# yassram/iterative-closest-point

Measured on AMD Instinct MI355X. Metric: ICP iterations/sec (synthetic 1048576-point pair, C4, exact NN), higher is better.
Workload: dtype f64 (30 exact fp64 grid searches (fp32 screen, candidates decided in fp64: the first from cell seeds, the seeded ones the fused grid iteration nn_grid_iter2_kernel, 75% of its queries kept their correspondence by the exclusion certificate without a walk); fp64 transform and reductions)

## Files before the change

### iterative-closest-point_amd/csrc/icp_canon.hip

```cpp
#include <hip/hip_runtime.h>

#include <cstdlib>

#include "icp_bundle_rec.h"
#include "icp_canon.h"
#include "icp_device.h"
#include "icp_fold.h"
#include "icp_gridbox.h"
#include "icp_kernels.h"
#include "icp_mfma16.h"

namespace icp {
namespace {

template <int K>
__device__ __forceinline__ void strands_to_row(const double (&acc)[K], double *__restrict__ rows, int R)
{
    __shared__ double sh[kBlock / 64][K];
    const int lane = threadIdx.x & 63, wave = threadIdx.x >> 6;
    if (lane == 0)
#pragma unroll
        for (int k = 0; k < K; ++k) sh[wave][k] = acc[k];
    __syncthreads();
    if (threadIdx.x < K) {
// ... 194 lines not shown
        const int k = threadIdx.x;
        double s[kFoldThreads / 64];
#pragma unroll
        for (int w = 0; w < kFoldThreads / 64; ++w) s[w] = sh[w][k];
#pragma unroll
        for (int span = 1; span < kFoldThreads / 64; span <<= 1)
#pragma unroll
            for (int w = 0; w < kFoldThreads / 64; w += 2 * span) s[w] = s[w] + s[w + span];
        sums[K0 + k] = s[0];
        s_sum[K0 + k] = s[0];
    }
    if (MODE == 0 && K0 == 0 && K == kCanonCols && threadIdx.x == 0)
        sums[kSumFar] = (double)__hip_atomic_load(&cs.s->far_acc, __ATOMIC_RELAXED, __HIP_MEMORY_SCOPE_AGENT);
    if constexpr (MODE == 0) return;
    __syncthreads();
    if (threadIdx.x != 0) return;
    if constexpr (MODE != 4)
        err_step_body(s_sum, cs.N, cs.threshold, cs.max_iter, cs.err_trace, cs.s, cs.hflag, cs.ticket, cs.h_state,
                      cs.h_trace);
    if constexpr (MODE == 1 || MODE == 4) horn_step_body(s_sum, cs.N, cs.c[0], cs.c[1], cs.c[2], 1, cs.cnt, cs.s);
}


template <int MODE>
__global__ __launch_bounds__(kFoldThreads) void canon_fold_cols_kernel(const double *__restrict__ rows, int R,
                                                                       double *__restrict__ sums, CanonStep cs, int S)
{
    __shared__ double sh[kFoldThreads / 64];
    __shared__ double s_sum[kCanonCols];
    __shared__ int s_last;
    const int lane = threadIdx.x & 63, wave = threadIdx.x >> 6, k = blockIdx.x;
    const double *col = rows + (size_t)k * (S > 0 ? S : R);
    double a = 0.0;
    constexpr int U = 4;
    for (int r0 = threadIdx.x; r0 < R; r0 += U * kFoldThreads) {
        double v[U];
#pragma unroll
        for (int u = 0; u < U; ++u) {
            const int r = r0 + u * kFoldThreads;
            v[u] = r < R ? canon_row_value(col, S, r) : 0.0;
        }
#pragma unroll
        for (int u = 0; u < U; ++u)
            if (r0 + u * kFoldThreads < R) a = a + v[u];
    }
    const double w = wave_tree_halves(a);
    const double two = lane_value(w, 31) + lane_value(w, 63);
    if (lane == 0) sh[wave] = two;
    __syncthreads();
    if (threadIdx.x == 0) {
// ... 30 lines not shown
                          int n, double *yx, double *yy, double *yz, const IterState *st_dev, double *rows,
                          hipStream_t st, const int *kpos, const double4 *m4kd, bool y_ready)
{
    if (n <= 0) return;
    const int R = canon_rows((size_t)n);
    if (y_ready)
        canon_moments_kernel<true><<<R, kBlock, 0, st>>>(idx, m4, px, py, pz, n, yx, yy, yz, st_dev, rows, kpos, m4kd);
    else
        canon_moments_kernel<false><<<R, kBlock, 0, st>>>(idx, m4, px, py, pz, n, yx, yy, yz, st_dev, rows, kpos, m4kd);
}

void launch_canon_transform(double *px, double *py, double *pz, const double *yx, const double *yy, const double *yz,
                            int n, const Xform *xf, const int *done, float4 *p32, double *rows, const SeedArgs &sa,
                            hipStream_t st)
{
    if (n <= 0) return;
    const int R = canon_rows((size_t)n);
    if (sa.qop)
        canon_transform_kernel<true><<<R, kBlock, 0, st>>>(px, py, pz, yx, yy, yz, n, xf, done, p32, rows, sa);
    else
        canon_transform_kernel<false><<<R, kBlock, 0, st>>>(px, py, pz, yx, yy, yz, n, xf, done, p32, rows, sa);
}

void launch_canon_fold(const double *rows, int n, double *sums, int mode, const CanonStep &cs, hipStream_t st,
                       int strands)
{
    const int R = canon_rows((size_t)(n > 0 ? n : 1));
    static const bool one = [] {
        const char *e = getenv("ICP_FOLD_ONE");
        return e && atoi(e) == 1;
    }();
    if (!one && cs.fold_ticket && (mode == 0 || mode == 1 || mode == 4)) {
        if (mode == 0) canon_fold_cols_kernel<0><<<kCanonCols, kFoldThreads, 0, st>>>(rows, R, sums, cs, strands);
        else if (mode == 1) canon_fold_cols_kernel<1><<<kCanonCols, kFoldThreads, 0, st>>>(rows, R, sums, cs, strands);
        else canon_fold_cols_kernel<4><<<kCanonCols, kFoldThreads, 0, st>>>(rows, R, sums, cs, strands);
        return;
    }
    switch (mode) {
    case 0: canon_fold_kernel<0, kCanonCols, 0><<<1, kFoldThreads, 0, st>>>(rows, R, sums, cs, strands); break;
    case 1: canon_fold_kernel<0, kCanonCols, 1><<<1, kFoldThreads, 0, st>>>(rows, R, sums, cs, strands); break;
    case 4: canon_fold_kernel<0, kCanonCols, 4><<<1, kFoldThreads, 0, st>>>(rows, R, sums, cs, strands); break;
    case 2: canon_fold_kernel<kSumErr, 1, 2><<<1, kFoldThreads, 0, st>>>(rows, R, sums, cs, strands); break;
    default: canon_fold_kernel<kSumErr, 1, 0><<<1, kFoldThreads, 0, st>>>(rows, R, sums, cs, strands); break;
    }
}

}
```

### iterative-closest-point_amd/csrc/icp_engine.h

```cpp
#pragma once

#include <hip/hip_runtime.h>
#include <rccl/rccl.h>

#include <string>
#include <vector>

#include "icp_canon.h"
#include "icp_kernels.h"

namespace icp {
namespace engine {

struct DevCloud {
    double *x = nullptr, *y = nullptr, *z = nullptr;
    float4 *f = nullptr;
    size_t n = 0, cap = 0;
};

}
}

using namespace icp;
using namespace icp::engine;
// ... 236 lines not shown
    bool seedd = false;
    int seed16 = 0;
    bool records = false;
    double rec_local = -1.0;
};

struct RunKnobs {
    int grid_budget;
    bool grid_auto, grid_iter;
    int grid_xcd;
    bool bundle_order_off, scene_order_off, cell_seed, first_k1;
    int run_mode;
    bool persist_mid_off, persist_stamps;
    int persist_cull;
    bool mid_prepass, transform_records;
    int far_shift;
    bool far_dist;
    int fused_steps;
    bool err_pair;
    int timing_stride;
    bool canon, cert;
    int cert_two;
    double cert_skin, cert_skin1;
    int iter_debug;
    bool tail_split_err, debug_policy;
};
const RunKnobs &run_knobs();

struct RunTestKnobs {
    int enqueue_delay_us;
    bool tail_test_abort, persist_test_abort;
};
RunTestKnobs run_test_knobs();

constexpr int kSeededBox = 125;

int fail(icp_ctx *ctx, int code, const std::string &msg);

template <class T> int grow(icp_ctx *ctx, T **p, size_t *cap, size_t count)
{
    if (*cap >= count && *p) return ICP_OK;
    if (*p) HIPCHK(hipFree(*p));
    *p = nullptr;
    *cap = 0;
    size_t bytes = sizeof(T) * (count ? count : 1);
    HIPCHK(hipMalloc((void **)p, bytes));
// ... 28 lines not shown
```

### iterative-closest-point_amd/csrc/icp_grid.hip

```cpp
#include <hip/hip_runtime.h>

#include <algorithm>
#include <cmath>
#include <cstdlib>
#include <string>
#include <type_traits>

#include "icp_canon.h"
#include "icp_device.h"
#include "icp_gridbox.h"
#include "icp_kernels.h"

namespace icp {
namespace {

__device__ __forceinline__ double d64g(double px, double py, double pz, double mx, double my,
                                       double mz)
{
    const double dx = px - mx;
    const double dy = py - my;
    const double dz = pz - mz;
    return (dx * dx + dy * dy) + dz * dz;
}

// ... 449 lines not shown
        best = d;
        bi = mi;
        bk = k;
    }
}

template <int G> __device__ __forceinline__ void group_lex_min_pos(double &best, int &bi, int &bk)
{
#pragma unroll
    for (int o = G / 2; o >= 1; o >>= 1) {
        const double ob = __shfl_xor(best, o, G);
        const int oi = __shfl_xor(bi, o, G);
        const int ok = __shfl_xor(bk, o, G);
        if (ob < best || (ob == best && (unsigned)oi < (unsigned)bi)) {
            best = ob;
            bi = oi;
            bk = ok;
        } else if (ob == best && oi == bi) {
            bk = max(bk, ok);
        }
    }
}

__device__ __forceinline__ int xcd_row(int b, int nb, int L)
{
    const int k = b & 7, i = b >> 3;
    if (L < 0) {
        const int q = nb >> 3, e = nb & 7;
        return k * q + min(k, e) + i;
    }
    if (L == 0 || b >= nb / (8 * L) * (8 * L)) return b;
    return ((i / L) * 8 + k) * L + i % L;
}

template <int G, int KR, int KU, int W, int TB = kBlock>
__global__ __launch_bounds__(TB, W) void nn_grid_seeded_kernel(
    int n, const double *__restrict__ px, const double *__restrict__ py, const double *__restrict__ pz, GridView gv,
    int budget, const double *__restrict__ seedd, const double4 *__restrict__ m4, int *__restrict__ idx,
    double *__restrict__ yx, double *__restrict__ yy, double *__restrict__ yz, int *far_count,
    int *__restrict__ far_list, int *__restrict__ far_hint, const int *__restrict__ stop, int xcd_remap, int trim)
{
    if (stop && *stop) return;
    const int sub = threadIdx.x & (G - 1);
    const int groups = gridDim.x * (TB / G);
    const int bx = xcd_row((int)blockIdx.x, (int)gridDim.x, xcd_remap);
    for (int t = (bx * TB + threadIdx.x) / G; t < n; t += groups) {
        const int h = idx[t];
        const double q[3] = {px[t], py[t], pz[t]};
        double best = seedd[t];
        int bi = h, bk = -1, c0[3], c1[3];
        const bool ok = h >= 0 && best == best && best < INFINITY && complete_box(q, best, gv, budget, c0, c1);
        if (ok) {
            const int ny = c1[1] - c0[1] + 1;
            const int nrows = ny * (c1[2] - c0[2] + 1);
            for (int r0 = sub; r0 < nrows; r0 += KR * G) {
                int k0[KR], pre[KR + 1];
// ... 748 lines not shown
    auto *p = (const ICP_CONST_AS IterState *)st;
    asm volatile("" : "+s"(p));
    return *(const IterState *)p;
}

template <bool A32, class T> __device__ __forceinline__ T &at32(T *b, int i)
{
    if constexpr (A32) return *(T *)((char *)b + (unsigned)i * (unsigned)sizeof(T));
    else return b[i];
}

template <int KR, int KU, int CH, int NWG, bool A32>
__global__ __launch_bounds__(64 * NWG) __attribute__((amdgpu_waves_per_eu(ICP_ITER2_WAVES))) void nn_grid_iter2_kernel(
    Iter2Args args_)
{
    static_assert(CH == 1 || CH == 2, "one or two chunks a task");
    constexpr bool kDbg = ICP_ITER2_DBG != 0;
    unsigned long long dcnt[4] = {0, 0, 0, 0};
    static_assert(NWG == 4 || NWG == 1, "a row or a strand a workgroup");
    constexpr int NW = NWG, QL = 2 / CH;
    __shared__ double s_tile[NW][CH * kIter2Tile];
    const Iter2Args &T = iter2_args();
    const IterState *const st = T.st;
    if (iter2_state(st).done) return;
    const int n = T.n, xcd_l = T.xcd_l, xform = T.xform;
    const int lane = threadIdx.x & 63, wave = threadIdx.x >> 6, u = lane / QL, sub = lane % QL;
    const int C = canon_chunks((size_t)n), S = canon_strands((size_t)n), R = canon_rows((size_t)n);
    const int s = NWG == 4 ? xcd_row((int)blockIdx.x, R, xcd_l) * 4 + wave
                           : xcd_row((int)blockIdx.x, S, xcd_l > 0 ? 4 * xcd_l : xcd_l);
    const int wr = s >> 2;
    double *const tile = s_tile[wave];
    double *const slots = tile;
    int *const wl = (int *)(tile + 32 * CH * kIter2Slot);
    auto at = [](auto *b, int i) -> auto & { return at32<A32>(b, i); };
    const bool cert_on = T.ca.state != nullptr, cert_in = cert_on && T.ca.valid != 0, two = T.ca.two != 0;
    auto wave_sync = [] {
        __builtin_amdgcn_fence(__ATOMIC_RELEASE, "wavefront");
        __builtin_amdgcn_wave_barrier();
        __builtin_amdgcn_fence(__ATOMIC_ACQUIRE, "wavefront");
    };
    double acc = 0.0;
    int far = 0, nbig = 0, ncert = 0, nwalk = 0;
    auto slot_t = [&](int c, int uu) { return (c + (uu >> 5) * S) * kCanonChunk + (uu & 31); };
    for (int c = s; s < S && c < C; c += CH * S) {
        const int t = slot_t(c, u);
        const bool active = c + (u >> 5) * S < C && t < n;
        if (kDbg) dcnt[0] += 1;
        const Iter2Args &A = iter2_args();
        const Xform xf = iter2_state(st).xf;
        double *const px = A.px, *const py = A.py, *const pz = A.pz, *const yx = A.yx, *const yy = A.yy, *const yz = A.yz;
        int *const idx = A.idx;
        int4 *const cstate = A.ca.state;
// ... 417 lines not shown
        wave_sync();
        double tv = 0.0;
        if ((lane & 31) < kCanonCols && (CH == 2 || lane < 32)) {
            const double *col = tile + (lane >> 5) * kIter2Tile + (lane & 31) * kLeafStride;
            double part[4];
#pragma unroll
            for (int g8 = 0; g8 < 4; ++g8) {
                double v[8];
#pragma unroll
                for (int j = 0; j < 8; ++j) v[j] = col[8 * g8 + j];
                part[g8] = ((v[0] + v[1]) + (v[2] + v[3])) + ((v[4] + v[5]) + (v[6] + v[7]));
            }
            tv = (part[0] + part[1]) + (part[2] + part[3]);
        }
        const double tb = CH == 2 ? __shfl(tv, (lane & 31) + 32, 64) : 0.0;
        if (lane < kCanonCols) {
            acc = acc + tv;
            if (CH == 2 && c + S < C) acc = acc + tb;
        }
        wave_sync();
    }
    const Iter2Args &E = iter2_args();
    unsigned long long *const dbg = E.dbg;
    if (kDbg && dbg && lane == 0)
        for (int f = 0; f < 4; ++f)
            if (dcnt[f]) atomicAdd(dbg + f, dcnt[f]);
    if constexpr (NWG == 4) {
        __shared__ double sh[NW][kCanonCols];
        if (lane < kCanonCols) sh[wave][lane] = acc;
        __syncthreads();
        if (threadIdx.x < kCanonCols) {
            const int k = threadIdx.x;
            E.rows[(size_t)k * R + wr] = (sh[0][k] + sh[1][k]) + (sh[2][k] + sh[3][k]);
        }
    } else if (s < S && lane < kCanonCols) {
        E.rows[(size_t)lane * S + s] = acc;
    }
    __shared__ int s_cnt[4][NW];
    for (int o = 32; o >= 1; o >>= 1) {
        far += __shfl_xor(far, o, 64);
        ncert += __shfl_xor(ncert, o, 64);
        nwalk += __shfl_xor(nwalk, o, 64);
    }
    if (lane == 0) {
        s_cnt[0][wave] = far;
        s_cnt[1][wave] = nbig;
        s_cnt[2][wave] = ncert;
        s_cnt[3][wave] = nwalk;
    }
    __syncthreads();
    if (threadIdx.x < 4) {
        int tot = 0;
        for (int w = 0; w < NW; ++w) tot += s_cnt[threadIdx.x][w];
        if (threadIdx.x < 2) {
            int *dst = threadIdx.x == 0 ? E.far_acc : E.big_count;
            if (tot && dst) atomicAdd(dst, tot);
        } else if (E.ca.counts && (NWG == 4 || s < S)) {
            E.ca.counts[2 * (NWG == 4 ? wr : s) + (threadIdx.x - 2)] += (unsigned long long)tot;
        }
    }
}

bool iter2_addr32(int n, int nm, const GridView &gv)
{
    const long long ncell = (long long)gv.g[0] * gv.g[1] * gv.g[2];
    return n <= (1 << 28) && nm <= (1 << 27) && ncell < (1ll << 30);
}

}

bool launch_nn_grid_iter(int n, double *px, double *py, double *pz, double *yx, double *yy, double *yz, int *idx,
                         const IterState *st_dev, float4 *p32, const GridView &gv, int box, int budget, int nm,
                         const double4 *m4, double *rows, int *far_acc, double far_d2, int *big_count, hipStream_t st,
                         unsigned long long *dbg, int xform, const CertArgs &ca, int *strands)
{
    if (strands) *strands = 0;
    if (n <= 0) return false;
    static const bool stage = [] {
        const char *e = getenv("ICP_ITER_STAGE");
        return e && atoi(e) == 1;
    }();
    static const bool wide_on = [] {
        const char *e = getenv("ICP_ITER_WIDE");
        return e && atoi(e) == 1;
    }();
    const int R = canon_rows((size_t)n);
    static const int xcd_env = [] {
        const char *e = getenv("ICP_ITER_XCD_L");
        return e ? atoi(e) : -2;
    }();
    const int xcd_l = xcd_env != -2 ? xcd_env : (canon_chunks((size_t)n) >= 8192 ? 32 : -1);
    static const bool v2 = [] {
        const char *e = getenv("ICP_ITER_V2");
        return !(e && e[0] == '0');
    }();
    if (v2 && !stage && !(wide_on && n <= kIterWideMax) && (!dbg || ICP_ITER2_DBG)) {
        static const int ch = [] {
            const char *e = getenv("ICP_ITER2_CH");
            return e && atoi(e) == 1 ? 1 : 2;
        }();
        static const int nwg = [] {
            const char *e = getenv("ICP_ITER2_NWG");
            return e && atoi(e) == 4 ? 4 : ICP_ITER2_NWG_DEFAULT;
        }();
        const int S = canon_strands((size_t)n);
        if (strands) *strands = nwg == 1 ? S : 0;
        const Iter2Args ka{n,      px, py, pz,   yx,      yy,     yz,        idx,   st_dev, p32, gv, box,
                           budget, nm, m4, rows, far_acc, far_d2, big_count, xform, xcd_l,  ca,  dbg};
        static const bool a32_on = [] {
            const char *e = getenv("ICP_ITER2_A32");
            return !(e && e[0] == '0');
        }();
        const bool a32 = a32_on && iter2_addr32(n, nm, gv);
        auto launch = [&](auto chc, auto nwgc, auto a32c) {
// ... 383 lines not shown
```

### iterative-closest-point_amd/csrc/icp_kernels.h

```cpp
#pragma once

#include <hip/hip_runtime.h>

#include "icp_internal.h"

namespace icp {

#if defined(__HIP_DEVICE_COMPILE__) || defined(__HIPCC__)
__device__ __forceinline__ int wave_append(int *counter, bool pred)
{
    const unsigned long long mask = __ballot(pred);
    if (mask == 0ull) return -1;
    const int lane = (int)(threadIdx.x & 63);
    const int leader = __ffsll((long long)mask) - 1;
    int base = 0;
    if (lane == leader) base = atomicAdd(counter, __popcll(mask));
    base = __shfl(base, leader, 64);
    return pred ? base + __popcll(mask & ((1ull << lane) - 1ull)) : -1;
}

__device__ __forceinline__ int block_append(int *counter, bool pred, int *counter2 = nullptr, bool pred2 = false)
{
    __shared__ int s_cnt[kBlock / 64], s_cnt2[kBlock / 64], s_base;
    const int lane = (int)(threadIdx.x & 63), wave = (int)(threadIdx.x >> 6);
// ... 316 lines not shown
    int queued2;
};

struct CanonStep {
    double N = 0.0;
    double threshold = 0.0;
    int max_iter = 0;
    double *err_trace = nullptr;
    IterState *s = nullptr;
    int *hflag = nullptr;
    int ticket = 0;
    IterState *h_state = nullptr;
    double *h_trace = nullptr;
    double c[3] = {0.0, 0.0, 0.0};
    int *cnt = nullptr;
    int *fold_ticket = nullptr;
};
void launch_canon_moments(const int *idx, const double4 *m4, const double *px, const double *py, const double *pz,
                          int n, double *yx, double *yy, double *yz, const IterState *st_dev, double *rows,
                          hipStream_t st, const int *kpos, const double4 *m4kd, bool y_ready);
void launch_canon_transform(double *px, double *py, double *pz, const double *yx, const double *yy, const double *yz,
                            int n, const Xform *xf, const int *done, float4 *p32, double *rows, const SeedArgs &sa,
                            hipStream_t st);
void launch_canon_fold(const double *rows, int n, double *sums, int mode, const CanonStep &cs, hipStream_t st,
                       int strands = 0);
struct GridView;
struct CertArgs {
    int4 *state = nullptr;
    int valid = 0;
    int two = 1;
    double skin = 0.0;
    unsigned long long *counts = nullptr;
};
bool launch_nn_grid_iter(int n, double *px, double *py, double *pz, double *yx, double *yy, double *yz, int *idx,
                         const IterState *st_dev, float4 *p32, const GridView &gv, int box, int budget, int nm,
                         const double4 *m4, double *rows, int *far_acc, double far_d2, int *big_count, hipStream_t st,
                         unsigned long long *dbg = nullptr,
                         int xform = 1,
                         const CertArgs &ca = CertArgs{},
                         int *strands = nullptr);
void launch_shifted_moments(const int *idx, const double4 *m4, const double *px, const double *py,
                            const double *pz, int n, double *yx, double *yy, double *yz, const IterState *st_dev,
                            double *partials, hipStream_t st, const int *kpos = nullptr,
                            const double4 *m4kd = nullptr, bool y_ready = false,
                            const StepFold &fold = StepFold{});
void launch_reduce_horn(const double *partials, int nblocks, double *sums, double n_total, const double c[3],
                        int shifted, int *amb_count, IterState *st_dev, hipStream_t st);
void launch_horn_step(const double *sums, double n_total, const double c[3], int shifted, int *amb_count,
                      IterState *st_dev, hipStream_t st);
void launch_err_horn_step(double *sums, double n_total, double threshold, int max_iter, double *err_trace,
                          IterState *st_dev, int *hflag_dev, int ticket, IterState *h_state_dev, double *h_trace_dev,
                          const double c[3], int shifted, int *amb_count, hipStream_t st,
                          int far_sum = 0);
void launch_err_step(double *sums, double n_total, double threshold, int max_iter, double *err_trace,
                     IterState *st_dev, int *hflag_dev, int ticket, IterState *h_state_dev, double *h_trace_dev,
                     hipStream_t st, const double *partials = nullptr, int nblocks = 0);
void launch_iteration_tail_small(const int *idx, const double4 *m4, double *px, double *py, double *pz, int n,
                                 double *yx, double *yy, double *yz, float4 *p32, double *sums, double n_total,
                                 const double c[3], int *amb_count, IterState *st_dev, double threshold,
                                 int max_iter, double *err_trace, int *hflag_dev, int ticket,
                                 IterState *h_state_dev, double *h_trace_dev, hipStream_t st);
constexpr size_t kPersistLdsMax = 160 * 1024 - 12 * 1024;
constexpr int kPersistMaxModel = (int)(kPersistLdsMax / 24);
// ... 132 lines not shown
```

### iterative-closest-point_amd/csrc/icp_run.hip

```cpp
#include <algorithm>
#include <chrono>
#include <cmath>
#include <cstdio>
#include <cstring>
#include <string>
#include <thread>
#include <vector>

#include "icp_engine.h"

namespace {

bool env_not0(const char *name)
{
    const char *e = getenv(name);
    return !(e && atoi(e) == 0);
}
bool env_first_not0(const char *name)
{
    const char *e = getenv(name);
    return !(e && e[0] == '0');
}
bool env_first1(const char *name)
{
    const char *e = getenv(name);
    return e && e[0] == '1';
}

RunKnobs read_run_knobs()
{
    RunKnobs k{};
    const char *e = getenv("ICP_GRID_BUDGET");
    k.grid_budget = e ? std::max(1, atoi(e)) : 0;
    k.grid_auto = env_not0("ICP_GRID_AUTO");
// ... 16 lines not shown
    e = getenv("ICP_PERSIST_NN");
    k.persist_cull = e && std::strcmp(e, "all") == 0 ? 0 : 1;
    k.mid_prepass = env_first1("ICP_MID_PREPASS");
    k.transform_records = env_not0("ICP_TRANSFORM_RECORDS");
    e = getenv("ICP_GRID_FAR_SHIFT");
    const int shift = e ? atoi(e) : 5;
    k.far_shift = shift >= 0 && shift <= 20 ? shift : 5;
    e = getenv("ICP_GRID_FAR");
    k.far_dist = e && std::string(e) == "dist";
    e = getenv("ICP_FUSED_STEPS");
    k.fused_steps = e ? atoi(e) & 3 : 0;
    k.err_pair = env_first_not0("ICP_ERR_PAIR");
    e = getenv("ICP_NN_TIMING_STRIDE");
    k.timing_stride = e ? std::max(1, atoi(e)) : 0;
    k.canon = env_first_not0("ICP_CANON");
    k.cert = env_first_not0("ICP_CERT");
    k.cert_two = env_first_not0("ICP_CERT_TWO") ? 1 : 0;
    e = getenv("ICP_CERT_SKIN");
    const double skin = e ? atof(e) : 0.25;
    k.cert_skin = skin >= 0.0 && skin <= 4.0 ? skin : 0.25;
    e = getenv("ICP_CERT_SKIN1");
    const double skin1 = e ? atof(e) : -1.0;
    k.cert_skin1 = skin1 >= 0.0 && skin1 <= 4.0 ? skin1 : k.cert_skin;
    e = getenv("ICP_ITER_DEBUG");
    k.iter_debug = !e ? 0 : atoi(e) == 2 ? 2 : 1;
    k.tail_split_err = getenv("ICP_TAIL_SPLIT_ERR") != nullptr;
    k.debug_policy = getenv("ICP_DEBUG_POLICY") != nullptr;
    return k;
}

struct KnobOwner {
    RunKnobs knobs;
    unsigned long long *iter_dbg;
};
KnobOwner &knob_owner()
{
    static KnobOwner o{read_run_knobs(), nullptr};
    return o;
}

}

const RunKnobs &icp::engine::run_knobs() { return knob_owner().knobs; }

RunTestKnobs icp::engine::run_test_knobs()
{
// ... 83 lines not shown
    RunTestKnobs tk{};
    bool need_p32 = false;
    bool fuse_seeds = false;
    bool lag = false;
    bool canon = false;
    bool grid_policy = false, carry = false, hold_first = false;
    int far_thr = 0;
    int far_obs = -1;
    int q2_obs = -1;
    int hold_far = -1;
    std::vector<int> fold_far;
    bool grid_next = false;
    bool fused_moments = false, fused_steps = false, err_pair = false, fused_tail = false, seeds_at_start = false;
    int tail_blocks = 0;
    unsigned tail_epoch = 0;
    const int *digest_order = nullptr;
    unsigned long long *iter_dbg = nullptr;
    SeedArgs sa;
    SeedArgs sa_grid;
    SeedState ws;
    CanonStep cs;
    CertArgs cert;
    bool cert_prev = false;
    bool xf_pending = false;
    int rows_strands = 0;
    int slot_ticket[kRing] = {};
    bool ar_timed[kRing] = {};
    int enqueued = 0, waited = 0, recorded = 0;
    bool stop = false;
    int timing_stride = 0, timing_phase = 0;
};

bool is_timed(const LoopRun &r, int it)
{
    return r.timing_stride > 0 && it % r.timing_stride == r.timing_phase && (it > 0 || r.timing_stride == 1);
}

int wait_one(LoopRun &r)
{
    icp_ctx *ctx = r.ctx;
    const int slot = r.waited % kRing;
    TRY(wait_flag(ctx, ctx->h_flags + 4 * slot + 2, r.slot_ticket[slot]));
    ++r.waited;
    if (r.grid_policy) {
        r.far_obs = ctx->h_iter->far_acc;
        if (r.waited - 1 < (int)r.fold_far.size()) r.fold_far[r.waited - 1] = r.far_obs;
// ... 549 lines not shown
    icp_ctx *ctx = r.ctx;
    const size_t n = r.n;
    const RunKnobs &k = run_knobs();
    DevCloud &P = ctx->scene;
    IterState *sd = ctx->iter_state;
    r.canon = k.canon && ctx->scene_slot && n > 0;
    if (r.canon) {
        TRY(grow(ctx, &ctx->canon_rowbuf, &ctx->canon_rowbuf_cap, (size_t)canon_strands(n) * kCanonCols));
        if (!ctx->h_far) HIPCHK(hipHostMalloc((void **)&ctx->h_far, sizeof(int), hipHostMallocDefault));
        launch_sum3(P.x, P.y, P.z, (int)n, red_target(ctx, n, ctx->sums + kSumScene), ctx->st, 1);
        red_finish(ctx, n, 3, ctx->sums + kSumScene);
        LAUNCHCHK("scene_sum");
        TRY(allreduce(ctx, ctx->sums + kSumScene, 3));
        if (k.first_k1) {
            launch_first_shift(sd, ctx->sums + kSumScene, r.N, ctx->st);
            LAUNCHCHK("first_shift");
        }
    }
    if (r.canon && k.cert && k.grid_iter && ctx->g_pts32) {
        TRY(grow(ctx, &ctx->cert_state, &ctx->cert_state_cap, n));
        const int crows = canon_strands(n);
        if (ctx->cert_counts_rows != crows) {
            TRY(fold_cert_counts(ctx));
            TRY(grow(ctx, &ctx->cert_counts, &ctx->cert_counts_cap, 2 * (size_t)crows));
            HIPCHK(hipMemsetAsync(ctx->cert_counts, 0, 2 * (size_t)crows * sizeof(ctx->cert_counts[0]), ctx->st));
            ctx->cert_counts_rows = crows;
        }
        r.cert.state = ctx->cert_state;
        r.cert.two = k.cert_two;
        r.cert.skin = k.cert_skin / ctx->grid.inv_h;
        r.cert.counts = ctx->cert_counts;
    }
    if (k.iter_debug && r.canon) {
        unsigned long long *&buf = knob_owner().iter_dbg;
        if (!buf) HIPCHK(hipMalloc((void **)&buf, 16 * sizeof(unsigned long long)));
        HIPCHK(hipMemsetAsync(buf, 0, 16 * sizeof(unsigned long long), ctx->st));
        r.iter_dbg = buf;
    }
    r.cs.N = r.N;
    r.cs.threshold = r.threshold;
    r.cs.max_iter = r.max_iter;
    r.cs.err_trace = ctx->err_trace_dev;
    r.cs.s = sd;
    r.cs.h_state = ctx->d_iter_mirror;
    r.cs.h_trace = ctx->d_trace;
    for (int a = 0; a < 3; ++a) r.cs.c[a] = ctx->c[a];
    r.cs.cnt = ctx->amb_count;
    if (!ctx->canon_ticket) {
        HIPCHK(hipMalloc((void **)&ctx->canon_ticket, sizeof(int)));
        HIPCHK(hipMemsetAsync(ctx->canon_ticket, 0, sizeof(int), ctx->st));
    }
    r.cs.fold_ticket = ctx->canon_ticket;
    return ICP_OK;
}

int run_setup(LoopRun &r, icp_ctx *ctx, int max_iter, double threshold, double *err_trace, icp_result *res,
              bool no_tail, bool *handed)
{
// ... 14 lines not shown
    }
    *handed = false;
    TRY(run_setup_policy(r));
    launch_run_init(ctx->iter_state, ctx->amb_count, ctx->st, ctx->c);
    TRY(run_setup_steps(r, no_tail));
    return run_setup_canon(r);
}


int canon_transform(LoopRun &r, const SeedArgs &sa_t)
{
    icp_ctx *ctx = r.ctx;
    DevCloud &P = ctx->scene, &Y = ctx->Y;
    IterState *sd = ctx->iter_state;
    launch_canon_transform(P.x, P.y, P.z, Y.x, Y.y, Y.z, (int)r.n, &sd->xf, &sd->done, r.need_p32 ? P.f : nullptr,
                           ctx->canon_rowbuf, sa_t, ctx->st);
    LAUNCHCHK("canon_transform");
    if (!r.need_p32) ctx->p32_stale = true;
    r.ws = seed_state_of(sa_t);
    r.xf_pending = false;
    return ICP_OK;
}

int canon_end(LoopRun &r, int it, bool horn, int slot)
{
    icp_ctx *ctx = r.ctx;
    IterState *sd = ctx->iter_state;
    CanonStep &cs = r.cs;
    const int sl = it % kRing;
    r.slot_ticket[sl] = ++ctx->flag_ticket;
    cs.hflag = ctx->d_flags + 4 * sl;
    cs.ticket = r.slot_ticket[sl];
    const int strands = r.rows_strands;
    r.rows_strands = 0;
    if (!r.lag) {
        launch_canon_fold(ctx->canon_rowbuf, (int)r.n, ctx->sums, horn ? 1 : 2, cs, ctx->st, strands);
        LAUNCHCHK("canon_fold");
        return ICP_OK;
    }
    launch_canon_fold(ctx->canon_rowbuf, (int)r.n, ctx->sums, horn ? 0 : 3, cs, ctx->st, strands);
    LAUNCHCHK("canon_fold");
    const bool tm = horn && slot >= 0 && r.ar_timed[slot];
    if (tm) HIPCHK(hipEventRecord(ctx->iter_ev[5 * slot + 3], ctx->st));
    TRY(horn ? allreduce(ctx, ctx->sums, r.grid_policy ? kNumSums + 1 : kNumSums)
             : allreduce(ctx, ctx->sums + kSumErr, 1));
    if (tm) HIPCHK(hipEventRecord(ctx->iter_ev[5 * slot + 4], ctx->st));
    if (horn)
        launch_err_horn_step(ctx->sums, r.N, r.threshold, r.max_iter, ctx->err_trace_dev, sd, cs.hflag, cs.ticket,
                             ctx->d_iter_mirror, ctx->d_trace, ctx->c, 1, ctx->amb_count, ctx->st,
                             r.grid_policy ? 1 : 0);
    else
        launch_err_step(ctx->sums, r.N, r.threshold, r.max_iter, ctx->err_trace_dev, sd, cs.hflag, cs.ticket,
                        ctx->d_iter_mirror, ctx->d_trace, ctx->st, nullptr, 0);
    LAUNCHCHK("err_step");
    return ICP_OK;
}

int canon_first(LoopRun &r)
{
    icp_ctx *ctx = r.ctx;
    const int strands = r.rows_strands;
    r.rows_strands = 0;
    if (!r.lag) {
        launch_canon_fold(ctx->canon_rowbuf, (int)r.n, ctx->sums, 4, r.cs, ctx->st, strands);
        LAUNCHCHK("canon_fold");
        return ICP_OK;
    }
    launch_canon_fold(ctx->canon_rowbuf, (int)r.n, ctx->sums, 0, r.cs, ctx->st, strands);
    LAUNCHCHK("canon_fold");
    TRY(allreduce(ctx, ctx->sums, kNumSums));
    launch_horn_step(ctx->sums, r.N, ctx->c, true, ctx->amb_count, ctx->iter_state, ctx->st);
    LAUNCHCHK("horn_step");
    return ICP_OK;
}

int finish_canon(LoopRun &r)
{
    TRY(canon_transform(r, r.grid_policy ? r.sa_grid : SeedArgs{}));
    return canon_end(r, r.enqueued - 1, false, -1);
}

int canon_tail(LoopRun &r, int slot, bool timed)
{
    if (r.enqueued == 0) {
        TRY(canon_first(r));
    } else {
        r.ar_timed[slot] = timed && r.lag;
        TRY(canon_end(r, r.enqueued - 1, true, slot));
    }
    r.xf_pending = true;
    ++r.enqueued;
    if (r.enqueued == r.max_iter) TRY(finish_canon(r));
    return ICP_OK;
}

int canon_path(LoopRun &r, bool *grid_out)
{
    icp_ctx *ctx = r.ctx;
    const int far_dec = r.enqueued >= 3 ? r.fold_far[r.enqueued - 3] : r.hold_far >= 0 ? r.hold_far : r.carry ? ctx->last_far : -1;
    bool grid_c = r.grid_policy && (far_dec >= 0 ? far_dec <= r.far_thr : r.enqueued == 0 ? r.grid_next : ctx->bundle_pending);
    if (r.xf_pending && r.hold_first && r.enqueued == 1 && far_dec < 0) {
        TRY(canon_transform(r, r.sa_grid));
        HIPCHK(hipMemcpyAsync(ctx->h_far, &ctx->iter_state->far_acc, sizeof(int), hipMemcpyDeviceToHost, ctx->st));
        HIPCHK(hipStreamSynchronize(ctx->st));
        r.hold_far = *ctx->h_far;
        if (r.lag) TRY(global_count(ctx, &r.hold_far));
        r.far_obs = r.hold_far;
        grid_c = r.hold_far <= r.far_thr;
    }
    *grid_out = grid_c;
    return ICP_OK;
}

void launch_fused_iter(LoopRun &r, int xform)
{
    icp_ctx *ctx = r.ctx;
    DevCloud &P = ctx->scene, &Y = ctx->Y;
    IterState *sd = ctx->iter_state;
    r.cert_prev = launch_nn_grid_iter((int)r.n, P.x, P.y, P.z, Y.x, Y.y, Y.z, ctx->idx, sd, r.need_p32 ? P.f : nullptr,
                                      grid_view(ctx), kSeededBox, grid_budget(ctx), (int)ctx->nm, ctx->m4,
                                      ctx->canon_rowbuf, r.grid_policy ? &sd->far_acc : nullptr,
                                      r.sa_grid.far_box > 0 ? -1.0 : r.sa_grid.far_d2, ctx->amb_count + 2, ctx->st,
                                      r.iter_dbg, xform, r.cert, &r.rows_strands);
}

int enqueue_canon_first_k1(LoopRun &r, int slot, bool timed)
{
    icp_ctx *ctx = r.ctx;
    const size_t n = r.n;
    DevCloud &P = ctx->scene, &Y = ctx->Y;
    TRY(grow(ctx, &ctx->idx, &ctx->idx_cap, n));
    launch_nn_grid_cell_seed((int)n, P.x, P.y, P.z, grid_view(ctx), (int)ctx->nm, ctx->idx, nullptr, ctx->st, Y.x, Y.y,
                             Y.z);
    LAUNCHCHK("nn_grid_cell_seed");
    if (timed) HIPCHK(hipEventRecord(ctx->iter_ev[5 * slot], ctx->st));
    r.cert.valid = 0;
    r.cert.skin = run_knobs().cert_skin1 / ctx->grid.inv_h;
    launch_fused_iter(r, 0);
    LAUNCHCHK("nn_grid_iter (first)");
    if (timed) HIPCHK(hipEventRecord(ctx->iter_ev[5 * slot + 1], ctx->st));
    r.ws = SeedState{};
    TRY(after_search(r, r.enqueued, true, slot));
    return canon_tail(r, slot, false);
}

int enqueue_canon_fused(LoopRun &r, int slot, bool timed)
{
    icp_ctx *ctx = r.ctx;
    const RunKnobs &k = run_knobs();
    if (timed) HIPCHK(hipEventRecord(ctx->iter_ev[5 * slot], ctx->st));
    r.cert.valid = r.cert_prev ? 1 : 0;
    r.cert.skin = (r.cert_prev ? k.cert_skin : k.cert_skin1) / ctx->grid.inv_h;
    launch_fused_iter(r, 1);
    if (r.iter_dbg && k.iter_debug == 2) {
        unsigned long long h[16];
        HIPCHK(hipStreamSynchronize(ctx->st));
        HIPCHK(hipMemcpy(h, r.iter_dbg, sizeof(h), hipMemcpyDeviceToHost));
        fprintf(stderr, "[iter2_debug] it %d tasks %llu walkers %llu batches %llu pair tests %llu (lane 0's)\n",
                r.enqueued, h[0], h[1], h[2], h[3]);
        HIPCHK(hipMemset(r.iter_dbg, 0, sizeof(h)));
    }
    LAUNCHCHK("nn_grid_iter");
    if (timed) HIPCHK(hipEventRecord(ctx->iter_ev[5 * slot + 1], ctx->st));
    if (!r.need_p32) ctx->p32_stale = true;
    r.ws = SeedState{};
    r.xf_pending = false;
    TRY(after_search(r, r.enqueued, true, slot));
    return canon_tail(r, slot, timed);
}

int enqueue_canon_search(LoopRun &r, int slot, bool timed, bool grid_c)
{
    icp_ctx *ctx = r.ctx;
    const size_t n = r.n;
    DevCloud &P = ctx->scene, &Y = ctx->Y;
    IterState *sd = ctx->iter_state;
    r.cert_prev = false;
    if (r.xf_pending) {
        SeedArgs sa_t = grid_c ? r.sa_grid : r.sa;
        if (!grid_c) records_args(r, sa_t);
        TRY(canon_transform(r, sa_t));
    }
    const double *gs = r.ws.seedd && (grid_c || ctx->nn_variant == ICP_NN_VARIANT_GRID) ? r.sa.seedd : nullptr;
    ctx->second_pass_items = r.grid_policy && r.q2_obs >= 0 ? std::max(256, 4 * r.q2_obs) : 0;
    TRY(nn_search_begin(ctx, P, n, ctx->seeds_valid, timed ? ctx->iter_ev[5 * slot] : nullptr,
                        timed ? ctx->iter_ev[5 * slot + 1] : nullptr, false, &r.ws, &sd->done, ctx->scene_slot, grid_c,
                        gs));
    TRY(after_search(r, r.enqueued, false, slot));
    if (r.enqueued == 0) {
        launch_first_shift_y_sample(ctx->idx, ctx->m4, Y.x, Y.y, Y.z, (int)n, ctx->kpos_valid ? ctx->kpos : nullptr,
                                    ctx->m4kd, ctx->y_ready, ctx->sums + kSumYSample, r.lag ? nullptr : sd,
                                    ctx->sums + kSumScene, r.N, ctx->st);
        LAUNCHCHK("first_shift_y_sample");
        if (r.lag) {
            TRY(allreduce(ctx, ctx->sums + kSumYSample, 4));
            launch_first_shifts(sd, ctx->sums + kSumYSample, ctx->sums + kSumScene, r.N, ctx->st);
            LAUNCHCHK("first_shifts");
        }
    }
    launch_canon_moments(ctx->idx, ctx->m4, P.x, P.y, P.z, (int)n, Y.x, Y.y, Y.z, sd, ctx->canon_rowbuf, ctx->st,
// ... 255 lines not shown
```

Baseline: 10410.

## Reorder iter2 strand dispatch by previous walk counts to balance load

The fused grid iteration now records, per strand, how many queries needed a walk in the previous iteration. Extra blocks in the fold kernel use those counts to build a block-to-strand order: a per-segment counting sort, with segments themselves ranked by total cost in the default form. The iteration kernel then reads its strand from this order, so heavy strands are dispatched first and the tail of the grid is less imbalanced. The cost is extra fold blocks, an extra scalar load per block, and a one-iteration-stale ordering heuristic.

```diff
diff --git a/iterative-closest-point_amd/csrc/icp_canon.hip b/iterative-closest-point_amd/csrc/icp_canon.hip
--- a/iterative-closest-point_amd/csrc/icp_canon.hip
+++ b/iterative-closest-point_amd/csrc/icp_canon.hip
@@ -240,10 +240,103 @@
 }
 
 
+constexpr int kOrderSlotsMax = kCanonStrandsMax / 8 + 1;
+constexpr int kOrderKeys = 65;
+
+__device__ __forceinline__ void order_wave_sync()
+{
+    __builtin_amdgcn_fence(__ATOMIC_RELEASE, "wavefront");
+    __builtin_amdgcn_wave_barrier();
+    __builtin_amdgcn_fence(__ATOMIC_ACQUIRE, "wavefront");
+}
+
+__device__ __forceinline__ void iter_order_build(const IterOrder &o, int k)
+{
+    constexpr int NW = kFoldThreads / 64;
+    __shared__ unsigned char s_key[kOrderSlotsMax];
+    __shared__ int s_base[NW][kOrderKeys + 1];
+    __shared__ int s_tot[kOrderSlotsMax];
+    const int lane = threadIdx.x & 63, wave = threadIdx.x >> 6;
+    const int S = o.S, L = o.L, form = o.form & 3;
+    const bool light = (o.form & 4) != 0;
+    const int nbij = L > 0 ? S / (8 * L) * (8 * L) : S;
+    const int nslots = L > 0 ? nbij / 8 : (S - k + 7) / 8;
+    if (S > kCanonStrandsMax || nslots > kOrderSlotsMax) return;
+    for (int b = nbij + k + 8 * (int)threadIdx.x; b < S; b += 8 * kFoldThreads) o.order[b] = b;
+    if (nslots <= 0) return;
+    const int seglen = L > 0 && form != 3 ? L : nslots, nseg = nslots / seglen;
+    for (int i = threadIdx.x; i < nslots; i += kFoldThreads) {
+        const int c = min(max(o.walk_last[xcd_row(8 * i + k, S, L)], 0), kOrderKeys - 1);
+        s_key[i] = (unsigned char)(light ? c : kOrderKeys - 1 - c);
+    }
+    __syncthreads();
+    if (form == 2) {
+        for (int seg = wave; seg < nseg; seg += NW) {
+            int t = 0;
+            for (int i = lane; i < seglen; i += 64) t += s_key[seg * seglen + i];
+            for (int d = 32; d >= 1; d >>= 1) t += __shfl_xor(t, d, 64);
+            if (lane == 0) s_tot[seg] = t;
+        }
+        __syncthreads();
+    }
+    for (int seg = wave; seg < nseg; seg += NW) {
+        int place = seg;
+        if (form == 2) {
+            const int mine = s_tot[seg];
+            int cnt = 0;
+            for (int j = lane; j < nseg; j += 64) {
+                const int tj = s_tot[j];
+                cnt += tj < mine || (tj == mine && j < seg) ? 1 : 0;
+            }
+            for (int d = 32; d >= 1; d >>= 1) cnt += __shfl_xor(cnt, d, 64);
+            place = cnt;
+        }
+        const int src = seg * seglen, dst = place * seglen;
+        int *const base = s_base[wave];
+        base[lane] = 0;
+        if (lane < kOrderKeys + 1 - 64) base[64 + lane] = 0;
+        order_wave_sync();
+        for (int i0 = 0; i0 < seglen; i0 += 64)
+            if (i0 + lane < seglen) atomicAdd(&base[s_key[src + i0 + lane]], 1);
+        order_wave_sync();
+        int incl = base[lane];
+        for (int d = 1; d < 64; d <<= 1) {
+            const int up = __shfl_up(incl, d, 64);
+            if (lane >= d) incl += up;
+        }
+        order_wave_sync();
+        base[lane + 1] = incl;
+        if (lane == 0) base[0] = 0;
+        order_wave_sync();
+        for (int i0 = 0; i0 < seglen; i0 += 64) {
+            const int i = i0 + lane;
+            const bool act = i < seglen;
+            const int key = act ? (int)s_key[src + i] : 127;
+            unsigned long long same = ~0ull;
+#pragma unroll
+            for (int bit = 0; bit < 7; ++bit) {
+                const unsigned long long bal = __ballot((key >> bit) & 1);
+                same &= (key >> bit) & 1 ? bal : ~bal;
+            }
+            const int before = __popcll(same & ((1ull << lane) - 1ull));
+            const int pos = act ? base[key] + before : 0;
+            order_wave_sync();
+            if (act && before == 0) base[key] = pos + __popcll(same);
+            order_wave_sync();
+            if (act) o.order[8 * (dst + pos) + k] = xcd_row(8 * (src + i) + k, S, L);
+        }
+    }
+}
+
 template <int MODE>
 __global__ __launch_bounds__(kFoldThreads) void canon_fold_cols_kernel(const double *__restrict__ rows, int R,
-                                                                       double *__restrict__ sums, CanonStep cs, int S)
-{
+                                                                       double *__restrict__ sums, CanonStep cs, int S,
+                                                                       IterOrder ord)
+{
+    if (blockIdx.x >= kCanonCols) {
+        iter_order_build(ord, (int)blockIdx.x - kCanonCols);
+        return;
+    }
     __shared__ double sh[kFoldThreads / 64];
     __shared__ double s_sum[kCanonCols];
     __shared__ int s_last;
@@ -320,8 +413,8 @@
         canon_transform_kernel<false><<<R, kBlock, 0, st>>>(px, py, pz, yx, yy, yz, n, xf, done, p32, rows, sa);
 }
 
-void launch_canon_fold(const double *rows, int n, double *sums, int mode, const CanonStep &cs, hipStream_t st,
-                       int strands)
+bool launch_canon_fold(const double *rows, int n, double *sums, int mode, const CanonStep &cs, hipStream_t st,
+                       int strands, const IterOrder &ord)
 {
     const int R = canon_rows((size_t)(n > 0 ? n : 1));
     static const bool one = [] {
@@ -329,10 +422,12 @@
         return e && atoi(e) == 1;
     }();
     if (!one && cs.fold_ticket && (mode == 0 || mode == 1 || mode == 4)) {
-        if (mode == 0) canon_fold_cols_kernel<0><<<kCanonCols, kFoldThreads, 0, st>>>(rows, R, sums, cs, strands);
-        else if (mode == 1) canon_fold_cols_kernel<1><<<kCanonCols, kFoldThreads, 0, st>>>(rows, R, sums, cs, strands);
-        else canon_fold_cols_kernel<4><<<kCanonCols, kFoldThreads, 0, st>>>(rows, R, sums, cs, strands);
-        return;
+        const bool build = ord.order && ord.walk_last && ord.form != 0 && ord.S > 0 && ord.S <= kCanonStrandsMax;
+        const int nb = kCanonCols + (build ? 8 : 0);
+        if (mode == 0) canon_fold_cols_kernel<0><<<nb, kFoldThreads, 0, st>>>(rows, R, sums, cs, strands, ord);
+        else if (mode == 1) canon_fold_cols_kernel<1><<<nb, kFoldThreads, 0, st>>>(rows, R, sums, cs, strands, ord);
+        else canon_fold_cols_kernel<4><<<nb, kFoldThreads, 0, st>>>(rows, R, sums, cs, strands, ord);
+        return build;
     }
     switch (mode) {
     case 0: canon_fold_kernel<0, kCanonCols, 0><<<1, kFoldThreads, 0, st>>>(rows, R, sums, cs, strands); break;
@@ -341,6 +436,7 @@
     case 2: canon_fold_kernel<kSumErr, 1, 2><<<1, kFoldThreads, 0, st>>>(rows, R, sums, cs, strands); break;
     default: canon_fold_kernel<kSumErr, 1, 0><<<1, kFoldThreads, 0, st>>>(rows, R, sums, cs, strands); break;
     }
-}
-
-}
+    return false;
+}
+
+}
diff --git a/iterative-closest-point_amd/csrc/icp_engine.h b/iterative-closest-point_amd/csrc/icp_engine.h
--- a/iterative-closest-point_amd/csrc/icp_engine.h
+++ b/iterative-closest-point_amd/csrc/icp_engine.h
@@ -282,6 +282,7 @@
     bool canon, cert;
     int cert_two;
     double cert_skin, cert_skin1;
+    int iter2_order;
     int iter_debug;
     bool tail_split_err, debug_policy;
 };
diff --git a/iterative-closest-point_amd/csrc/icp_grid.hip b/iterative-closest-point_amd/csrc/icp_grid.hip
--- a/iterative-closest-point_amd/csrc/icp_grid.hip
+++ b/iterative-closest-point_amd/csrc/icp_grid.hip
@@ -495,16 +495,6 @@
     }
 }
 
-__device__ __forceinline__ int xcd_row(int b, int nb, int L)
-{
-    const int k = b & 7, i = b >> 3;
-    if (L < 0) {
-        const int q = nb >> 3, e = nb & 7;
-        return k * q + min(k, e) + i;
-    }
-    if (L == 0 || b >= nb / (8 * L) * (8 * L)) return b;
-    return ((i / L) * 8 + k) * L + i % L;
-}
 
 template <int G, int KR, int KU, int W, int TB = kBlock>
 __global__ __launch_bounds__(TB, W) void nn_grid_seeded_kernel(
@@ -1299,12 +1289,22 @@
     __shared__ double s_tile[NW][CH * kIter2Tile];
     const Iter2Args &T = iter2_args();
     const IterState *const st = T.st;
-    if (iter2_state(st).done) return;
+    const unsigned long long dbg_t0 = kDbg ? __builtin_amdgcn_s_memrealtime() : 0ull;
+    const int *const ord = NWG == 1 ? T.ca.order : nullptr;
+    auto *oaddr = ord ? (const ICP_CONST_AS int *)ord + blockIdx.x : (const ICP_CONST_AS int *)&st->done;
+    auto *daddr = (const ICP_CONST_AS int *)&st->done;
+    int s_ord, done;
+    asm volatile("s_load_dword %0, %2, 0x0\n\ts_load_dword %1, %3, 0x0\n\ts_waitcnt lgkmcnt(0)"
+                 : "=&s"(done), "=&s"(s_ord)
+                 : "s"(daddr), "s"(oaddr)
+                 : "memory");
+    if (done) return;
     const int n = T.n, xcd_l = T.xcd_l, xform = T.xform;
     const int lane = threadIdx.x & 63, wave = threadIdx.x >> 6, u = lane / QL, sub = lane % QL;
     const int C = canon_chunks((size_t)n), S = canon_strands((size_t)n), R = canon_rows((size_t)n);
     const int s = NWG == 4 ? xcd_row((int)blockIdx.x, R, xcd_l) * 4 + wave
-                           : xcd_row((int)blockIdx.x, S, xcd_l > 0 ? 4 * xcd_l : xcd_l);
+                : ord ? ((unsigned)s_ord < (unsigned)S ? s_ord : S)
+                      : xcd_row((int)blockIdx.x, S, xcd_l > 0 ? 4 * xcd_l : xcd_l);
     const int wr = s >> 2;
     double *const tile = s_tile[wave];
     double *const slots = tile;
@@ -1768,7 +1768,7 @@
     }
     const Iter2Args &E = iter2_args();
     unsigned long long *const dbg = E.dbg;
-    if (kDbg && dbg && lane == 0)
+    if (kDbg && dbg && lane == 0 && NWG != 1)
         for (int f = 0; f < 4; ++f)
             if (dcnt[f]) atomicAdd(dbg + f, dcnt[f]);
     if constexpr (NWG == 4) {
@@ -1793,6 +1793,15 @@
         s_cnt[1][wave] = nbig;
         s_cnt[2][wave] = ncert;
         s_cnt[3][wave] = nwalk;
+        if (NWG == 1 && E.ca.walk_last && s < S) E.ca.walk_last[s] = nwalk;
+        if (kDbg && dbg && NWG == 1) {
+            unsigned long long *const rec = dbg + 16 + 4 * (size_t)blockIdx.x;
+            rec[0] = dbg_t0;
+            rec[1] = __builtin_amdgcn_s_memrealtime();
+            rec[2] = (unsigned long long)(unsigned)s << 32 | (unsigned long long)(blockIdx.x & 7) << 16 |
+                     (unsigned long long)(nwalk & 0xffff);
+            rec[3] = (dcnt[0] & 0xffffull) << 48 | (dcnt[2] & 0xffffull) << 32 | (dcnt[3] & 0xffffffffull);
+        }
     }
     __syncthreads();
     if (threadIdx.x < 4) {
@@ -1813,6 +1822,21 @@
     return n <= (1 << 28) && nm <= (1 << 27) && ncell < (1ll << 30);
 }
 
+}
+
+static int iter_xcd_l(int n)
+{
+    static const int xcd_env = [] {
+        const char *e = getenv("ICP_ITER_XCD_L");
+        return e ? atoi(e) : -2;
+    }();
+    return xcd_env != -2 ? xcd_env : (canon_chunks((size_t)n) >= 8192 ? 32 : -1);
+}
+
+int nn_grid_iter_strand_run(int n)
+{
+    const int xcd_l = iter_xcd_l(n);
+    return xcd_l > 0 ? 4 * xcd_l : xcd_l;
 }
 
 bool launch_nn_grid_iter(int n, double *px, double *py, double *pz, double *yx, double *yy, double *yz, int *idx,
@@ -1831,11 +1855,7 @@
         return e && atoi(e) == 1;
     }();
     const int R = canon_rows((size_t)n);
-    static const int xcd_env = [] {
-        const char *e = getenv("ICP_ITER_XCD_L");
-        return e ? atoi(e) : -2;
-    }();
-    const int xcd_l = xcd_env != -2 ? xcd_env : (canon_chunks((size_t)n) >= 8192 ? 32 : -1);
+    const int xcd_l = iter_xcd_l(n);
     static const bool v2 = [] {
         const char *e = getenv("ICP_ITER_V2");
         return !(e && e[0] == '0');
diff --git a/iterative-closest-point_amd/csrc/icp_kernels.h b/iterative-closest-point_amd/csrc/icp_kernels.h
--- a/iterative-closest-point_amd/csrc/icp_kernels.h
+++ b/iterative-closest-point_amd/csrc/icp_kernels.h
@@ -362,8 +362,24 @@
 void launch_canon_transform(double *px, double *py, double *pz, const double *yx, const double *yy, const double *yz,
                             int n, const Xform *xf, const int *done, float4 *p32, double *rows, const SeedArgs &sa,
                             hipStream_t st);
-void launch_canon_fold(const double *rows, int n, double *sums, int mode, const CanonStep &cs, hipStream_t st,
-                       int strands = 0);
+__host__ __device__ inline int xcd_row(int b, int nb, int L)
+{
+    const int k = b & 7, i = b >> 3;
+    if (L < 0) {
+        const int q = nb >> 3, e = nb & 7;
+        return k * q + (k < e ? k : e) + i;
+    }
+    if (L == 0 || b >= nb / (8 * L) * (8 * L)) return b;
+    return ((i / L) * 8 + k) * L + i % L;
+}
+struct IterOrder {
+    const int *walk_last = nullptr;
+    int *order = nullptr;
+    int S = 0, L = 0, form = 0;
+};
+bool launch_canon_fold(const double *rows, int n, double *sums, int mode, const CanonStep &cs, hipStream_t st,
+                       int strands = 0,
+                       const IterOrder &ord = IterOrder{});
 struct GridView;
 struct CertArgs {
     int4 *state = nullptr;
@@ -371,6 +387,8 @@
     int two = 1;
     double skin = 0.0;
     unsigned long long *counts = nullptr;
+    int *walk_last = nullptr;
+    const int *order = nullptr;
 };
 bool launch_nn_grid_iter(int n, double *px, double *py, double *pz, double *yx, double *yy, double *yz, int *idx,
                          const IterState *st_dev, float4 *p32, const GridView &gv, int box, int budget, int nm,
@@ -379,6 +397,7 @@
                          int xform = 1,
                          const CertArgs &ca = CertArgs{},
                          int *strands = nullptr);
+int nn_grid_iter_strand_run(int n);
 void launch_shifted_moments(const int *idx, const double4 *m4, const double *px, const double *py,
                             const double *pz, int n, double *yx, double *yy, double *yz, const IterState *st_dev,
                             double *partials, hipStream_t st, const int *kpos = nullptr,
diff --git a/iterative-closest-point_amd/csrc/icp_run.hip b/iterative-closest-point_amd/csrc/icp_run.hip
--- a/iterative-closest-point_amd/csrc/icp_run.hip
+++ b/iterative-closest-point_amd/csrc/icp_run.hip
@@ -10,6 +10,11 @@
 #include "icp_engine.h"
 
 namespace {
+
+#ifndef ICP_ITER2_DBG
+#define ICP_ITER2_DBG 0
+#endif
+constexpr size_t kIterDbgRec = ICP_ITER2_DBG ? 4 * (size_t)icp::kCanonStrandsMax : 0;
 
 bool env_not0(const char *name)
 {
@@ -72,6 +77,8 @@
     e = getenv("ICP_CERT_SKIN1");
     const double skin1 = e ? atof(e) : -1.0;
     k.cert_skin1 = skin1 >= 0.0 && skin1 <= 4.0 ? skin1 : k.cert_skin;
+    e = getenv("ICP_ITER2_ORDER");
+    k.iter2_order = !e ? 2 : atoi(e) >= 1 && atoi(e) <= 7 && atoi(e) != 4 ? atoi(e) : 0;
     e = getenv("ICP_ITER_DEBUG");
     k.iter_debug = !e ? 0 : atoi(e) == 2 ? 2 : 1;
     k.tail_split_err = getenv("ICP_TAIL_SPLIT_ERR") != nullptr;
@@ -201,6 +208,8 @@
     CanonStep cs;
     CertArgs cert;
     bool cert_prev = false;
+    IterOrder order;
+    bool walk_written = false, order_ok = false;
     bool xf_pending = false;
     int rows_strands = 0;
     int slot_ticket[kRing] = {};
@@ -796,18 +805,26 @@
         const int crows = canon_strands(n);
         if (ctx->cert_counts_rows != crows) {
             TRY(fold_cert_counts(ctx));
-            TRY(grow(ctx, &ctx->cert_counts, &ctx->cert_counts_cap, 2 * (size_t)crows));
-            HIPCHK(hipMemsetAsync(ctx->cert_counts, 0, 2 * (size_t)crows * sizeof(ctx->cert_counts[0]), ctx->st));
+            TRY(grow(ctx, &ctx->cert_counts, &ctx->cert_counts_cap, 3 * (size_t)crows));
+            HIPCHK(hipMemsetAsync(ctx->cert_counts, 0, 3 * (size_t)crows * sizeof(ctx->cert_counts[0]), ctx->st));
             ctx->cert_counts_rows = crows;
         }
         r.cert.state = ctx->cert_state;
         r.cert.two = k.cert_two;
         r.cert.skin = k.cert_skin / ctx->grid.inv_h;
         r.cert.counts = ctx->cert_counts;
+        if (k.iter2_order) {
+            r.cert.walk_last = (int *)(ctx->cert_counts + 2 * (size_t)crows);
+            r.order.walk_last = r.cert.walk_last;
+            r.order.order = r.cert.walk_last + crows;
+            r.order.S = crows;
+            r.order.L = nn_grid_iter_strand_run((int)n);
+            r.order.form = k.iter2_order;
+        }
     }
     if (k.iter_debug && r.canon) {
         unsigned long long *&buf = knob_owner().iter_dbg;
-        if (!buf) HIPCHK(hipMalloc((void **)&buf, 16 * sizeof(unsigned long long)));
+        if (!buf) HIPCHK(hipMalloc((void **)&buf, (16 + kIterDbgRec) * sizeof(unsigned long long)));
         HIPCHK(hipMemsetAsync(buf, 0, 16 * sizeof(unsigned long long), ctx->st));
         r.iter_dbg = buf;
     }
@@ -868,6 +885,13 @@
     return ICP_OK;
 }
 
+IterOrder fold_order(LoopRun &r)
+{
+    const bool build = r.walk_written;
+    r.walk_written = false;
+    return build ? r.order : IterOrder{};
+}
+
 int canon_end(LoopRun &r, int it, bool horn, int slot)
 {
     icp_ctx *ctx = r.ctx;
@@ -879,12 +903,13 @@
     cs.ticket = r.slot_ticket[sl];
     const int strands = r.rows_strands;
     r.rows_strands = 0;
+    const IterOrder ord = fold_order(r);
     if (!r.lag) {
-        launch_canon_fold(ctx->canon_rowbuf, (int)r.n, ctx->sums, horn ? 1 : 2, cs, ctx->st, strands);
+        r.order_ok = launch_canon_fold(ctx->canon_rowbuf, (int)r.n, ctx->sums, horn ? 1 : 2, cs, ctx->st, strands, ord);
         LAUNCHCHK("canon_fold");
         return ICP_OK;
     }
-    launch_canon_fold(ctx->canon_rowbuf, (int)r.n, ctx->sums, horn ? 0 : 3, cs, ctx->st, strands);
+    r.order_ok = launch_canon_fold(ctx->canon_rowbuf, (int)r.n, ctx->sums, horn ? 0 : 3, cs, ctx->st, strands, ord);
     LAUNCHCHK("canon_fold");
     const bool tm = horn && slot >= 0 && r.ar_timed[slot];
     if (tm) HIPCHK(hipEventRecord(ctx->iter_ev[5 * slot + 3], ctx->st));
@@ -907,12 +932,13 @@
     icp_ctx *ctx = r.ctx;
     const int strands = r.rows_strands;
     r.rows_strands = 0;
+    const IterOrder ord = fold_order(r);
     if (!r.lag) {
-        launch_canon_fold(ctx->canon_rowbuf, (int)r.n, ctx->sums, 4, r.cs, ctx->st, strands);
+        r.order_ok = launch_canon_fold(ctx->canon_rowbuf, (int)r.n, ctx->sums, 4, r.cs, ctx->st, strands, ord);
         LAUNCHCHK("canon_fold");
         return ICP_OK;
     }
-    launch_canon_fold(ctx->canon_rowbuf, (int)r.n, ctx->sums, 0, r.cs, ctx->st, strands);
+    r.order_ok = launch_canon_fold(ctx->canon_rowbuf, (int)r.n, ctx->sums, 0, r.cs, ctx->st, strands, ord);
     LAUNCHCHK("canon_fold");
     TRY(allreduce(ctx, ctx->sums, kNumSums));
     launch_horn_step(ctx->sums, r.N, ctx->c, true, ctx->amb_count, ctx->iter_state, ctx->st);
@@ -958,16 +984,46 @@
     return ICP_OK;
 }
 
+int dump_wave_records(LoopRun &r, unsigned long long cnt[4])
+{
+    if (!ICP_ITER2_DBG || r.rows_strands <= 0) return ICP_OK;
+    icp_ctx *ctx = r.ctx;
+    const size_t nb = (size_t)r.rows_strands;
+    std::vector<unsigned long long> h(4 + 4 * nb);
+    h[0] = 0x4c494154524554ull;
+    h[1] = (unsigned long long)r.enqueued;
+    h[2] = nb;
+    h[3] = r.n;
+    HIPCHK(hipMemcpy(h.data() + 4, r.iter_dbg + 16, 4 * nb * sizeof(h[0]), hipMemcpyDeviceToHost));
+    for (size_t b = 0; b < nb; ++b) {
+        const unsigned long long w = h[4 + 4 * b + 2], c = h[4 + 4 * b + 3];
+        cnt[0] += c >> 48;
+        cnt[1] += w & 0xffffull;
+        cnt[2] += (c >> 32) & 0xffffull;
+        cnt[3] += c & 0xffffffffull;
+    }
+    const char *path = getenv("ICP_ITER_TAIL_DUMP");
+    if (!path) return ICP_OK;
+    FILE *f = fopen(path, "ab");
+    if (!f) return fail(ctx, ICP_E_HIP, "ICP_ITER_TAIL_DUMP: cannot open the file");
+    fwrite(h.data(), sizeof(h[0]), h.size(), f);
+    fclose(f);
+    return ICP_OK;
+}
+
 void launch_fused_iter(LoopRun &r, int xform)
 {
     icp_ctx *ctx = r.ctx;
     DevCloud &P = ctx->scene, &Y = ctx->Y;
     IterState *sd = ctx->iter_state;
+    r.cert.order = r.order_ok ? r.order.order : nullptr;
+    r.order_ok = false;
     r.cert_prev = launch_nn_grid_iter((int)r.n, P.x, P.y, P.z, Y.x, Y.y, Y.z, ctx->idx, sd, r.need_p32 ? P.f : nullptr,
                                       grid_view(ctx), kSeededBox, grid_budget(ctx), (int)ctx->nm, ctx->m4,
                                       ctx->canon_rowbuf, r.grid_policy ? &sd->far_acc : nullptr,
                                       r.sa_grid.far_box > 0 ? -1.0 : r.sa_grid.far_d2, ctx->amb_count + 2, ctx->st,
                                       r.iter_dbg, xform, r.cert, &r.rows_strands);
+    r.walk_written = r.cert_prev && r.cert.valid && r.cert.walk_last && r.rows_strands == r.order.S;
 }
 
 int enqueue_canon_first_k1(LoopRun &r, int slot, bool timed)
@@ -1002,6 +1058,7 @@
         unsigned long long h[16];
         HIPCHK(hipStreamSynchronize(ctx->st));
         HIPCHK(hipMemcpy(h, r.iter_dbg, sizeof(h), hipMemcpyDeviceToHost));
+        TRY(dump_wave_records(r, h));
         fprintf(stderr, "[iter2_debug] it %d tasks %llu walkers %llu batches %llu pair tests %llu (lane 0's)\n",
                 r.enqueued, h[0], h[1], h[2], h[3]);
         HIPCHK(hipMemset(r.iter_dbg, 0, sizeof(h)));
@@ -1022,6 +1079,7 @@
     DevCloud &P = ctx->scene, &Y = ctx->Y;
     IterState *sd = ctx->iter_state;
     r.cert_prev = false;
+    r.walk_written = r.order_ok = false;
     if (r.xf_pending) {
         SeedArgs sa_t = grid_c ? r.sa_grid : r.sa;
         if (!grid_c) records_args(r, sa_t);
```

New measurement: 10700 (median of 6 runs). 1.03x the previous value.
